# Girjoaba/simplex_method_gpu

Hardware: AMD Instinct MI355X
Metric: simplex iterations/sec on dense m=4096 n=16384 fp64; achieved HBM GB/s (higher is better)
Workload: dtype f64

## Files before the change

include/simplex.h:

```cpp
#ifndef SIMPLEX_MI355X_H
#define SIMPLEX_MI355X_H

#include <stdint.h>

#ifdef __cplusplus
extern "C" {
#endif

#define SPX_ABI_VERSION 8

#define SPX_STATUS_MAX_ITER       0
#define SPX_STATUS_OPTIMUM_FOUND  1
#define SPX_STATUS_UNBOUNDED      2
#define SPX_STATUS_THETA_OVERFLOW 3
#define SPX_STATUS_INFEASIBLE     4

#define SPX_OK             0
#define SPX_ERR_ARG       -1
#define SPX_ERR_HIP       -2
#define SPX_ERR_OOM       -3
#define SPX_ERR_RCCL      -4
#define SPX_ERR_STATE     -5
#define SPX_ERR_NO_DEVICE -6
#define SPX_ERR_SINGULAR  -7
// ... 181 lines not shown

#define SPX_LOOP_FIELDS 7
int spx_loop_times(spx_ctx* ctx, double out[SPX_LOOP_FIELDS], int64_t* passes);

int spx_info(spx_ctx* ctx, int64_t* m, int64_t* n, int64_t* ld,
             int64_t* local_nonbasic, double* bytes_price, double* bytes_update);

#define SPX_CONFIG_FIELDS 17
int spx_config(spx_ctx* ctx, int32_t out[SPX_CONFIG_FIELDS]);

#define SPX_LOOP_LAYOUT_FIELDS 8
int spx_loop_layout(spx_ctx* ctx, int32_t out[SPX_LOOP_LAYOUT_FIELDS]);

int spx_ftran_cols(spx_ctx* ctx, int32_t* cols);

#define SPX_DISPATCH_FIELDS 10
int spx_dispatch_stats(spx_ctx* ctx, int64_t out[SPX_DISPATCH_FIELDS]);

int spx_prepare(spx_ctx* ctx);

int spx_shard_range(int64_t m, int64_t n, int32_t rank, int32_t nranks, int64_t out[4]);
int spx_minloc_merge(const double* vals, const int64_t* idx, int32_t count,
                     double* best_val, int64_t* best_idx);

const char* spx_last_error(void);
const char* spx_status_string(int32_t status);
int spx_abi_version(void);

#ifdef __cplusplus
}
#endif
// ... 2 lines not shown
```

simplex_method_gpu_amd/__init__.py:

```python
from __future__ import annotations

import ctypes
from dataclasses import dataclass
from enum import IntEnum
from typing import NamedTuple

import numpy as np

from ._lib import SimplexError, SpxOpts, check, load

__all__ = ["SolveStatus", "SolveResult", "Context", "solve", "read_lp", "comm_unique_id",
           "shard_range", "minloc_merge", "group_iterate", "group_sync", "check_ranks",
           "SimplexError", "FLAG_TIMING", "RATIO_REFERENCE", "RATIO_GUARDED", "RATIO_HARRIS",
           "PRICING_DANTZIG", "PRICING_DEVEX", "PRICING_STEEPEST", "ALGO_PRIMAL", "ALGO_DUAL",
           "DUAL_PRICING_DANTZIG", "DUAL_PRICING_STEEPEST", "FLAG_DUAL_STEEPEST",
           "DUAL_RATIO_TEXTBOOK", "DUAL_RATIO_LONG_STEP", "FLAG_DUAL_LONG_STEP", "ALGO_PRIMAL_BOX",
           "FLAG_PRIMAL_PHASE1", "PRIMAL_PRICING_DANTZIG", "PRIMAL_PRICING_STEEPEST", "FLAG_PRIMAL_STEEPEST",
           "PRIMAL_WEIGHTS_REFERENCE", "PRIMAL_WEIGHTS_EXACT", "FLAG_PRIMAL_EXACT_WEIGHTS",
           "CostRanging", "RhsRanging"]

FLAG_TIMING = 1
FLAG_STAMPS = 2
FLAG_GLOBAL_Y = 4
FLAG_ROW_SHARD = 8
# ... 496 lines not shown
    def info(self):
        m, n, ld, nb = ctypes.c_int64(), ctypes.c_int64(), ctypes.c_int64(), ctypes.c_int64()
        bp, bu = ctypes.c_double(), ctypes.c_double()
        check(self._L.spx_info(self._h, ctypes.byref(m), ctypes.byref(n), ctypes.byref(ld), ctypes.byref(nb),
                               ctypes.byref(bp), ctypes.byref(bu)))
        return {"m": m.value, "n": n.value, "ld": ld.value, "local_nonbasic": nb.value,
                "bytes_price": bp.value, "bytes_update": bu.value}


    def ftran_cols(self) -> int:
        v = ctypes.c_int32()
        check(self._L.spx_ftran_cols(self._h, ctypes.byref(v)))
        return v.value

    def dispatch_stats(self):
        out = (ctypes.c_int64 * 10)()
        check(self._L.spx_dispatch_stats(self._h, out))
        keys = ("eager_passes", "graph_launches", "graph_passes", "persistent_launches", "persistent_passes",
                "folds", "window_pos", "window", "persist_fallbacks", "graph_builds")
        return dict(zip(keys, list(out)))

    def config(self):
        out = (ctypes.c_int32 * 17)()
        check(self._L.spx_config(self._h, out))
        keys = ("window", "price_block", "price_grid", "price_lds", "update_block", "update_rows", "update_grid",
                "graph_batch", "persistent", "loop_block", "tableau", "loop_grid", "defer_tail", "compact_fold",
                "ftran_rows_per_wave", "mbox_fused", "compact_price")
        cfg = dict(zip(keys, list(out)))
        cfg["dual_pricing"] = self._dual_pricing
        cfg["primal_pricing"] = self._primal_pricing
        cfg["dual_ratio"] = self._dual_ratio
        cfg["primal_weights"] = self._primal_weights
        return cfg

    def loop_layout(self):
        out = (ctypes.c_int32 * 8)()
        check(self._L.spx_loop_layout(self._h, out))
        keys = ("dual_price_lds", "dual_update_lds", "dual_se_update_lds", "dual_se_rho_lds", "pbox_price_lds",
                "pbox_update_lds", "pbox_se_lds_vecs", "slack_unit")
        return dict(zip(keys, list(out)))


def solve(A_cols, b, c, max_iter: int = (1 << 62), eps: float = 1e-7, device: int = -1,
# ... 4 lines not shown
```

simplex_method_gpu_amd/csrc/spx_api.cpp:

```cpp
#include <algorithm>
#include <cmath>
#include <cstdarg>
#include <cstdio>
#include <cstdlib>
#include <cstring>
#include <string>
#include <vector>

#include "spx_ctx.h"
#include "spx_tableau.h"

using namespace spx;
using namespace spx_host;

namespace {

thread_local std::string g_err;

}

int spx_host::fail(int code, const char* fmt, ...) {
    char buf[512];
    va_list ap;
    va_start(ap, fmt);
// ... 403 lines not shown
    HIP_TRY(launch_reset(x->P, x->stream));
    SPX_TRY(box_sync(x));
    HIP_TRY(launch_se_init(x->P, x->stream));
    if (x->P.bc) {
        HIP_TRY(hipMemsetAsync(x->P.rleft, 0, (size_t)x->L * sizeof(int32_t), x->stream));
        HIP_TRY(hipMemsetAsync(x->P.rmap, 0xFF, (size_t)x->L * sizeof(int32_t), x->stream));
        HIP_TRY(hipMemsetAsync(x->P.bc_n, 0, BC_N_WORDS * sizeof(int32_t), x->stream));
        if (x->P.as_off) HIP_TRY(hipMemsetAsync(x->P.as_off, 0, 65 * sizeof(int32_t), x->stream));
    }
    SPX_TRY(tab_rebuild(x, true));
    HIP_TRY(hipStreamSynchronize(x->stream));
    x->pivots = 0;
    x->status = SPX_STATUS_MAX_ITER;
    x->stepped_price = false;
    x->nw = 0;
    x->dw_ok = false;
    x->s_list = 0;
    x->cp_now = x->cp_ok;
    return SPX_OK;
}

bool fold_due(const spx_ctx* x) { return x->P.win && x->nw >= x->P.win; }
void advance_window(spx_ctx* x, bool folded) {
    if (x->P.win) x->nw = (folded ? 1 : x->nw) + 1;
}

int fold_events(spx_ctx* x, hipEvent_t* f0, hipEvent_t* f1) {
    if (x->ev_fold.size() < 2 * (x->n_fold + 1)) {
        for (int i = 0; i < 2; ++i) {
            hipEvent_t e;
            HIP_TRY(hipEventCreate(&e));
// ... 8 lines not shown

int enqueue_pass(spx_ctx* x, bool timed) {
    hipEvent_t p0 = nullptr, p1 = nullptr, u0 = nullptr, u1 = nullptr;
    if (timed) SPX_TRY(pass_events(x, &p0, &p1, &u0, &u1));
    const bool fold = fold_due(x);
    if (x->capturing) x->graph_folds += fold ? 1 : 0;
    else {
        ++x->n_eager;
        x->n_folds += fold ? 1 : 0;
    }
    if (fold) {
        hipEvent_t f0 = nullptr, f1 = nullptr;
        if (timed) SPX_TRY(fold_events(x, &f0, &f1));
        if (x->defer_tail) HIP_TRY(launch_apply_tail(x->P, x->stream));
        if (f0) HIP_TRY(hipEventRecord(f0, x->stream));
        HIP_TRY(launch_fold(x->P, x->P.win, x->cus, x->stream));
        if (f1) HIP_TRY(hipEventRecord(f1, x->stream));
        x->dw_ok = false;
    }
    const bool cp_open = x->cp_now && !x->dw_ok && (fold || x->nw <= 1);
    const bool cp_pass = x->cp_now && x->dw_ok;
    advance_window(x, fold);
    HIP_TRY(launch_se_prep(x->P, x->stream, (x->se_fuse && x->se_chain && !fold) ? x->ucfg.grid : 0));
    Params Pp = x->P;
    Pp.se_fused = x->se_fuse ? 1 : 0;
    Pp.defer_price = x->defer_ok ? 1 : 0;
    Pp.defer_tail = x->defer_tail ? 1 : 0;
    Pp.mbox_fused = (x->mbox_ready && x->mbox_fused) ? 1 : 0;
    if (cp_pass) Pp.price_grid = x->ccfg.grid;
    HIP_TRY(launch_price(Pp, cp_pass ? x->ccfg : (cp_open ? x->dcfg : x->pcfg), x->stream, p0, p1));
    if (cp_open) {
        HIP_TRY(launch_dw_basic(Pp, x->stream));
        x->dw_ok = true;
    }
    if (x->use_comm) {
        if (x->mbox_ready) {
            if (!Pp.mbox_fused) HIP_TRY(launch_exchange(x->P, x->stream));
        } else {
            if (!x->comm_ready) return fail(SPX_ERR_STATE, "nranks > 1 but neither spx_attach_comm nor spx_mbox_attach was called");
            NCCL_TRY(ncclAllGather(x->send, x->recv, sizeof(ArgMinEntry) * x->P.pr_stride, ncclUint8, x->comm,
                                   x->stream));
        }
    }
    if (timed) HIP_TRY(hipEventRecord(x->ev_xend[x->n_price - 1], x->stream));
    HIP_TRY(launch_update(Pp, x->ucfg, x->stream, u0, u1));
    x->se_chain = x->se_fuse;
    if (x->P.split_tail) HIP_TRY(launch_tail(x->P, x->ucfg.grid, x->stream));
    if (x->P.row_shard) {
        if (!x->comm_ready) return fail(SPX_ERR_STATE, "row-sharded B^-1 needs spx_attach_comm");
        NCCL_TRY(ncclAllGather(x->P.rs_send, x->rs_recv, (size_t)x->P.rs_stride, ncclUint8, x->comm, x->stream));
        HIP_TRY(launch_finalize_rs(x->P, x->stream));
    }
    return SPX_OK;
}

int build_graph(spx_ctx* x) {
    hipGraphExec_t& gexec = x->cp_now ? x->graph_exec_c : x->graph_exec;
    hipGraph_t& gkeep = x->cp_now ? x->graph_c : x->graph;
    if (gexec || x->batch <= 0) return SPX_OK;
    if (x->use_comm && !x->comm_ready && !x->mbox_ready)
        return fail(SPX_ERR_STATE, "nranks > 1 but neither spx_attach_comm nor spx_mbox_attach was called");
    HIP_TRY(hipStreamBeginCapture(x->stream, hipStreamCaptureModeThreadLocal));
    int rc = SPX_OK;
    const int nw_keep = x->nw;
    const bool dw_keep = x->dw_ok;
    if (x->P.win) x->nw = x->P.win;
    x->capturing = true;
    x->graph_folds = 0;
    for (int i = 0; i < x->batch && rc == SPX_OK; ++i) rc = enqueue_pass(x, false);
    x->capturing = false;
    x->se_chain = false;
    x->nw = nw_keep;
    x->dw_ok = dw_keep;
    hipGraph_t g = nullptr;
    hipError_t e = hipStreamEndCapture(x->stream, &g);
    hipError_t ei = hipSuccess;
    if (rc == SPX_OK && e == hipSuccess) ei = hipGraphInstantiate(&gexec, g, nullptr, nullptr, 0);
    if (x->use_comm && (rc != SPX_OK || e != hipSuccess || ei != hipSuccess)) {
        if (g) (void)hipGraphDestroy(g);
        gexec = nullptr;
        x->batch = 0;
        x->graph_fallback = true;
        (void)hipGetLastError();
        return SPX_OK;
    }
    if (rc != SPX_OK) return rc;
    if (e != hipSuccess) return fail(SPX_ERR_HIP, "hipStreamEndCapture: %s", hipGetErrorString(e));
    gkeep = g;
    if (ei != hipSuccess) return fail(SPX_ERR_HIP, "hipGraphInstantiate: %s", hipGetErrorString(ei));
    ++x->n_graph_builds;
    HIP_TRY(hipGraphUpload(gexec, x->stream));
    HIP_TRY(hipStreamSynchronize(x->stream));
    return SPX_OK;
}

int build_graphs(spx_ctx* x) {
    if (!x->cp_ok) return build_graph(x);
    const bool keep = x->cp_now;
    const int64_t built = x->n_graph_builds;
    int rc = SPX_OK;
    for (int mode = 1; mode >= 0 && rc == SPX_OK; --mode) {
        x->cp_now = mode != 0;
        rc = build_graph(x);
    }
    x->cp_now = keep;
    if (x->n_graph_builds > built) x->n_graph_builds = built + 1;
    return rc;
}

int check_tickets(spx_ctx* x) {
    bool bad = x->st_host->uncovered != 0;
    if (!bad && x->P.price_dyn && (x->pcfg.wm == 2 || x->pcfg.tk)) {
        uint32_t t[TICKET_WORDS];
        HIP_TRY(hipMemcpy(t, x->P.tickets, sizeof(t), hipMemcpyDeviceToHost));
        for (int k = 0; k < 2 * x->P.tk_shards; ++k) bad = bad || t[32 * k + 1] > t[32 * k];
    }
    if (bad) {
        return fail(SPX_ERR_STATE, "pricing: ticketed list slots were left unpriced (tk_shards %d, grid %d): the "
// ... 119 lines not shown
    if (x->algo == SPX_ALGO_DUAL) return iterate_dual(x, k);
    if (x->algo == SPX_ALGO_PRIMAL_BOX) return iterate_pbox(x, k);
    if (x->persist && !x->stepped_price) {
        SPX_TRY(set_limit(x, x->pivots + k));
        return iterate_persist(x, k);
    }
    if (x->stepped_price) return fail(SPX_ERR_STATE, "spx_price was called without spx_pivot");
    if (!x->cp_ok) return iterate_passes(x, k);
    int64_t left = k;
    while (left > 0 && x->status == SPX_STATUS_MAX_ITER) {
        const int64_t room = (int64_t)x->P.as_cap - x->s_list - x->nw;
        const bool cp = room >= 16;
        const int64_t chunk = cp ? std::min(left, room) : left;
        if (cp != x->cp_now) {
            x->cp_now = cp;
            x->dw_ok = false;
        }
        const int64_t before = x->pivots;
        SPX_TRY(iterate_passes(x, chunk));
        left -= chunk;
        if (x->pivots == before) break;
    }
    return SPX_OK;
}

int iterate_passes(spx_ctx* x, int64_t k) {
    SPX_TRY(set_limit(x, x->pivots + k));
    x->se_chain = false;
    int64_t left = k;
    if (x->batch > 0) {
        const int64_t lead = x->P.win ? std::max(0, x->P.win - x->nw) : 0;
        if (left >= lead + x->batch) {
            for (int64_t i = 0; i < lead; ++i) SPX_TRY(enqueue_pass(x, x->timing));
            left -= lead;
            SPX_TRY(build_graph(x));
            hipGraphExec_t gexec = x->cp_now ? x->graph_exec_c : x->graph_exec;
            const int64_t reps = left / x->batch;
            for (int64_t i = 0; i < reps; ++i) HIP_TRY(hipGraphLaunch(gexec, x->stream));
            if (reps > 0 && x->cp_now) x->dw_ok = true;
            x->se_chain = false;
            x->n_graph_launch += reps;
            x->n_graph_pass += reps * x->batch;
            x->n_folds += reps * x->graph_folds;
            left -= reps * x->batch;
        }
    }
    for (int64_t i = 0; i < left; ++i) SPX_TRY(enqueue_pass(x, x->timing));
    if (x->defer_tail) HIP_TRY(launch_apply_tail(x->P, x->stream));
    x->se_chain = false;
    return read_state(x);
}

int rv_prepare(spx_ctx* x) {
    if (x->rv.X) return SPX_OK;
    RvParams& R = x->rv;
    const int64_t m = x->m, L = x->L;
    R.A = x->A;
    R.m = m;
// ... 64 lines not shown
        return fail(SPX_ERR_SINGULAR, "singular basis: no pivot above tolerance for column %lld (basis position %lld)",
                    (long long)basis[rs.bad_pos], (long long)rs.bad_pos);
    HIP_TRY(rv_launch_finish(x->P, R, x->rv_Ypart, x->stream));
    if (x->P.bc) {
        std::vector<int32_t> left((size_t)x->L, 0);
        for (int64_t k = 0; k < m; ++k) left[(size_t)k] = basis[k] != ns + k ? 1 : 0;
        HIP_TRY(hipMemcpyAsync(x->P.rleft, left.data(), (size_t)x->L * sizeof(int32_t), hipMemcpyHostToDevice,
                               x->stream));
        HIP_TRY(hipMemsetAsync(x->P.rmap, 0xFF, (size_t)x->L * sizeof(int32_t), x->stream));
        HIP_TRY(hipMemsetAsync(x->P.bc_n, 0, BC_N_WORDS * sizeof(int32_t), x->stream));
        HIP_TRY(launch_compact(x->P, x->stream));
        HIP_TRY(hipStreamSynchronize(x->stream));
    }
    SPX_TRY(tab_rebuild(x, false));
    x->nw = 0;
    x->dw_ok = false;
    dual_on_reinvert(x);
    SPX_TRY(pbox_on_reinvert(x));
    return read_state(x);
}

int check_basis(const spx_ctx* x, const int64_t* basis) {
    if (!basis) return fail(SPX_ERR_ARG, "basis is NULL");
    std::vector<char> seen((size_t)x->n, 0);
    for (int64_t k = 0; k < x->m; ++k) {
        const int64_t j = basis[k];
        if (j < 0 || j >= x->n) return fail(SPX_ERR_ARG, "basis[%lld] = %lld out of range", (long long)k, (long long)j);
        if (seen[(size_t)j]) return fail(SPX_ERR_ARG, "column %lld repeated in the basis", (long long)j);
        seen[(size_t)j] = 1;
    }
    return SPX_OK;
// ... 96 lines not shown
    cc.tk = false;
    cc.lds_bytes = (size_t)(cc.block / 64) * sizeof(PricePartial) + 16 + (size_t)round_up(cap, 2) * 16;
    x->dcfg = x->pcfg;
    x->dcfg.dw = true;
    int per_cu = 0, per_cu_d = 0;
    HIP_TRY(price_prepare(cc, &per_cu));
    HIP_TRY(price_prepare(x->dcfg, &per_cu_d));
    const int waves = cc.block / 64;
    cc.grid = (int)std::max<int64_t>(1, std::min<int64_t>({(x->max_local_cols + waves - 1) / waves,
                                                           (int64_t)x->cus * std::max(per_cu, 1), P.price_cap}));
    if (x->opts.price_grid > 0) cc.grid = (int)std::min<int64_t>(x->opts.price_grid, P.price_cap);
    P.as_ld = cap;
    P.as_cap = (int32_t)cap;
    P.AS = static_cast<double*>(d);
    x->cp_ok = x->cp_now = true;
    return SPX_OK;
}

int create_tail(spx_ctx* x) {
    SPX_TRY(do_reset(x));
    if (x->algo == SPX_ALGO_DUAL) return dual_setup(x);
    if (x->algo == SPX_ALGO_PRIMAL_BOX) return pbox_setup(x);
    if (!x->use_comm && !x->persist) SPX_TRY(build_graphs(x));
    return SPX_OK;
}

}

namespace spx_host {

// ... 50 lines not shown
    if (x->status == ST_HANDOFF_TIMEOUT) return fail(SPX_ERR_STATE, "internal error: ratio-test hand-off timed out");
    if (x->status == ST_CPRICE_STATE)
        return fail(SPX_ERR_STATE, "internal error: compact pricing without its rows of A or a valid dw (list %d, rows %d)",
                    x->s_list, x->P.as_cap);
    SPX_TRY(check_tickets(x));
    return SPX_OK;
}

int flush(spx_ctx* x) {
    if (x->stepped_price) return fail(SPX_ERR_STATE, "state readback between spx_price and spx_pivot");
    SPX_TRY(pbox_fresh_y(x));
    if (x->P.win) {
        HIP_TRY(launch_fold(x->P, 2, x->cus, x->stream));
        HIP_TRY(launch_tab_binv(x->P, x->stream));
        x->nw = std::min(x->nw, 1);
        x->dw_ok = false;
    }
    HIP_TRY(launch_flush(x->P, x->stream));
    return SPX_OK;
}

int set_limit(spx_ctx* x, int64_t limit) {
    *x->limit_host = limit;
    HIP_TRY(hipMemcpyAsync(&x->P.st->limit, x->limit_host, sizeof(int64_t), hipMemcpyHostToDevice, x->stream));
    return SPX_OK;
}

int set_running(spx_ctx* x) {
    SPX_TRY(read_state(x));
    const int32_t run = ST_RUNNING;
    HIP_TRY(hipMemcpy(&x->P.st->status, &run, sizeof(run), hipMemcpyHostToDevice));
// ... 57 lines not shown
        spx_destroy(x);
        g_err = keep;
        return rc;
    }
    *out = x;
    return SPX_OK;
}

void spx_destroy(spx_ctx* x) {
    if (!x) return;
    if (x->stream) (void)hipStreamSynchronize(x->stream);
    if (x->graph_exec) (void)hipGraphExecDestroy(x->graph_exec);
    if (x->graph) (void)hipGraphDestroy(x->graph);
    if (x->graph_exec_c) (void)hipGraphExecDestroy(x->graph_exec_c);
    if (x->graph_c) (void)hipGraphDestroy(x->graph_c);
    for (hipEvent_t e : {x->ev_sent, x->ev_recv, x->ev_sent2, x->ev_recv2})
        if (e) (void)hipEventDestroy(e);
    for (hipEvent_t e : x->ev_price) (void)hipEventDestroy(e);
    for (hipEvent_t e : x->ev_update) (void)hipEventDestroy(e);
    for (hipEvent_t e : x->ev_xend) (void)hipEventDestroy(e);
    for (hipEvent_t e : x->ev_loop) (void)hipEventDestroy(e);
    for (hipEvent_t e : x->ev_fold) (void)hipEventDestroy(e);
    for (hipEvent_t e : x->pbox.ev_vtb) (void)hipEventDestroy(e);
    for (hipEvent_t e : x->pbox.ev_wx) (void)hipEventDestroy(e);
    for (const std::vector<hipEvent_t>& v : x->rng.ev)
        for (hipEvent_t e : v) (void)hipEventDestroy(e);
    if (x->comm) (void)ncclCommDestroy(x->comm);
    for (void* p : x->mbox_opened) (void)hipIpcCloseMemHandle(p);
    for (void* p : x->allocs) (void)hipFree(p);
    if (x->st_host) (void)hipHostFree(x->st_host);
// ... 237 lines not shown
        }
    }
    if (cs[0]->status == SPX_STATUS_MAX_ITER && k > 0) {
        for (int g = 0; g < G; ++g) {
            HIP_TRY(hipSetDevice(cs[g]->device));
            SPX_TRY(set_limit(cs[g], cs[g]->pivots + k));
            cs[g]->se_chain = false;
        }
        for (int64_t it = 0; it < k; ++it) {
            for (int g = 0; g < G; ++g) {
                spx_ctx* x = cs[g];
                HIP_TRY(hipSetDevice(x->device));
                const bool fold = fold_due(x);
                if (fold && x->defer_tail) HIP_TRY(launch_apply_tail(x->P, x->stream));
                if (fold) HIP_TRY(launch_fold(x->P, x->P.win, x->cus, x->stream));
                advance_window(x, fold);
                HIP_TRY(launch_se_prep(x->P, x->stream, (x->se_fuse && x->se_chain && !fold) ? x->ucfg.grid : 0));
                ++x->n_eager;
                x->n_folds += fold ? 1 : 0;
                Params Pp = x->P;
                Pp.defer_tail = x->defer_tail ? 1 : 0;
                HIP_TRY(launch_price(Pp, x->pcfg, x->stream, nullptr, nullptr));
                HIP_TRY(hipEventRecord(x->ev_sent, x->stream));
            }
            for (int h = 0; h < G; ++h) {
                spx_ctx* x = cs[h];
                HIP_TRY(hipSetDevice(x->device));
                const int ps = x->P.pr_stride;
                for (int g = 0; g < G; ++g) {
                    HIP_TRY(hipStreamWaitEvent(x->stream, cs[g]->ev_sent, 0));
// ... 204 lines not shown
    if (z) SPX_TRY(spx_objective(x, z));
    SPX_TRY(spx_get_state(x, x_b, b_ixs, nullptr, nullptr, nullptr, status, pivots));
    return SPX_OK;
}

int spx_price(spx_ctx* x, int64_t* p, double* min_e, int32_t* optimal) {
    if (!x) return fail(SPX_ERR_ARG, "ctx is NULL");
    if (x->algo == SPX_ALGO_DUAL)
        return fail(SPX_ERR_STATE, "spx_price / spx_pivot step the primal loop only (the context runs SPX_ALGO_DUAL)");
    if (x->algo == SPX_ALGO_PRIMAL_BOX)
        return fail(SPX_ERR_STATE, "spx_price / spx_pivot step the primal loop only (the context runs SPX_ALGO_PRIMAL_BOX)");
    if (x->status != SPX_STATUS_MAX_ITER) return fail(SPX_ERR_STATE, "solve already terminated");
    SPX_TRY(set_limit(x, x->pivots + 1));
    const bool fold = fold_due(x);
    if (fold) HIP_TRY(launch_fold(x->P, x->P.win, x->cus, x->stream));
    if (fold) x->dw_ok = false;
    ++x->n_eager;
    x->n_folds += fold ? 1 : 0;
    HIP_TRY(launch_se_prep(x->P, x->stream));
    SPX_TRY(clear_tickets(x));
    HIP_TRY(launch_price(x->P, x->pcfg, x->stream, nullptr, nullptr));
    const int ps = x->P.pr_stride;
    if (x->use_comm) {
        if (x->mbox_ready) {
            HIP_TRY(launch_exchange(x->P, x->stream));
        } else {
            if (!x->comm_ready) return fail(SPX_ERR_STATE, "nranks > 1 but neither spx_attach_comm nor spx_mbox_attach was called");
            NCCL_TRY(ncclAllGather(x->send, x->recv, sizeof(ArgMinEntry) * ps, ncclUint8, x->comm, x->stream));
        }
    }
    std::vector<ArgMinEntry> cand((size_t)x->opts.nranks * ps);
// ... 36 lines not shown
    return SPX_OK;
}

int spx_dispatch_stats(spx_ctx* x, int64_t out[SPX_DISPATCH_FIELDS]) {
    if (!x || !out) return fail(SPX_ERR_ARG, "NULL argument");
    out[0] = x->n_eager;
    out[1] = x->n_graph_launch;
    out[2] = x->n_graph_pass;
    out[3] = x->n_persist_launch;
    out[4] = x->n_persist_pass;
    out[5] = x->n_folds;
    out[6] = x->P.win ? x->nw : 0;
    out[7] = x->P.win;
    out[8] = x->n_persist_fallback;
    out[9] = x->n_graph_builds;
    return SPX_OK;
}

int spx_prepare(spx_ctx* x) {
    if (!x) return fail(SPX_ERR_ARG, "ctx is NULL");
    if (x->persist) return SPX_OK;
    if (x->algo != SPX_ALGO_PRIMAL) return SPX_OK;
    return build_graphs(x);
}

int spx_pass_times(spx_ctx* x, double out[3], int64_t* passes) {
    if (!x || !out) return fail(SPX_ERR_ARG, "NULL argument");
    HIP_TRY(hipStreamSynchronize(x->stream));
    double tp = 0.0, tx = 0.0, tu = 0.0;
    for (size_t i = 0; i < x->n_price; ++i) {
// ... 97 lines not shown
    if (ld) *ld = x->L;
    if (local_nb) *local_nb = x->st_host->nb_count;
    int64_t streamed = x->st_host->nb_count;
    if (x->P.slack_unit) {
        std::vector<int64_t> bix((size_t)x->m);
        HIP_TRY(hipMemcpy(bix.data(), x->P.b_ixs, (size_t)x->m * sizeof(int64_t), hipMemcpyDeviceToHost));
        int64_t basic_slacks = 0;
        for (int64_t j : bix) basic_slacks += (j >= x->P.k_lo && j < x->P.k_hi) ? 1 : 0;
        streamed -= (x->P.k_hi - x->P.k_lo) - basic_slacks;
    }
    if (bp) *bp = 8.0 * (double)(x->m + 1) * (double)streamed;
    if (bp && x->cp_ok && x->cp_now && x->P.win > 2) {
        const double kw = (double)x->P.win;
        const double per_col = 8.0 * ((double)x->s_list + 2.0 + 0.5 * (kw - 1.0) + 1.0);
        const double compact = per_col * (double)x->st_host->nb_count;
        *bp = ((kw - 2.0) * compact + *bp) / (kw - 1.0);
    }
    int32_t cols = 0;
    SPX_TRY(spx_ftran_cols(x, &cols));
    const double md = (double)x->m;
    const double fold = (x->P.bc && x->P.cfold) ? 8.0 * md * (3.0 * cols + x->P.win) : 16.0 * md * md;
    if (bu) *bu = x->P.win ? 8.0 * md * (double)cols + fold / (x->P.win - 1) : 16.0 * md * md;
    return SPX_OK;
}

int spx_ftran_cols(spx_ctx* x, int32_t* cols) {
    if (!x || !cols) return fail(SPX_ERR_ARG, "NULL argument");
    *cols = (int32_t)x->m;
    if (x->P.win && x->P.bc) {
        HIP_TRY(hipStreamSynchronize(x->stream));
        HIP_TRY(hipMemcpy(cols, x->P.bc_n, sizeof(int32_t), hipMemcpyDeviceToHost));
    }
    return SPX_OK;
}

int spx_config(spx_ctx* x, int32_t out[SPX_CONFIG_FIELDS]) {
// ... 40 lines not shown
```

simplex_method_gpu_amd/csrc/spx_ctx.h:

```cpp
#pragma once
#include <hip/hip_runtime.h>
#include <rccl/rccl.h>

#include <algorithm>
#include <cstdint>
#include <vector>

#include "../../include/simplex.h"
#include "spx_device.h"
#include "spx_dual.h"
#include "spx_kernels.h"
#include "spx_loop.h"
#include "spx_pbox.h"
#include "spx_ranging.h"
#include "spx_reinv.h"

namespace spx_host {

int fail(int code, const char* fmt, ...);

}

#define HIP_TRY(expr)                                                                          \
    do {                                                                                       \
        hipError_t e_ = (expr);                                                                \
// ... 94 lines not shown
    bool graph_fallback = false;
    uint64_t* mbox = nullptr;
    uint32_t* mbox_seq = nullptr;
    uint64_t** mbox_peer = nullptr;
    std::vector<void*> mbox_opened;
    bool mbox_ready = false;
    bool mbox_fused = false;
    bool bc_want = false;
    bool slack_ident = false;
    bool defer_ok = false;
    bool defer_tail = false;
    bool se_fuse = false;
    bool se_chain = false;
    int64_t se_rows = 0;

    bool cp_ok = false, cp_now = false, dw_ok = false;
    spx::PriceCfg ccfg{}, dcfg{};
    int32_t s_list = 0;
    int32_t* bcn_host = nullptr;

    hipGraphExec_t graph_exec = nullptr;
    hipGraph_t graph = nullptr;
    hipGraphExec_t graph_exec_c = nullptr;
    hipGraph_t graph_c = nullptr;
    int batch = 0;

    hipEvent_t ev_sent = nullptr, ev_recv = nullptr, ev_sent2 = nullptr, ev_recv2 = nullptr;
    int64_t mb = 0;
    unsigned char* rs_recv = nullptr;

    bool timing = false;
    std::vector<hipEvent_t> ev_price, ev_update;
    std::vector<hipEvent_t> ev_xend;
    size_t n_price = 0, n_update = 0;

    int64_t pivots = 0;
    int32_t status = SPX_STATUS_MAX_ITER;
    bool stepped_price = false;
    int nw = 0;
// ... 88 lines not shown
```

simplex_method_gpu_amd/csrc/spx_foldk.hip:

```cpp
#include <hip/hip_runtime.h>
#include <math.h>

#include "spx_device.h"
#include "spx_common.h"
#include "spx_fold.h"
#include "spx_kernels.h"
#include "spx_tableau.h"

namespace spx {

template <int KW>
__global__ __launch_bounds__(FOLD_THREADS) void k_fold(Params P, int min_nw) {
    DevState* st = P.st;
    const int nw = st->nw;
    if (nw < min_nw || nw < 2) return;
    const int nf = nw - 1;
    __shared__ double Rl[KW][FOLD_RP];
    __shared__ double NT[KW][FOLD_NP<KW>];
    __shared__ int s_last;
    const int tid = threadIdx.x, lane = tid & 63;
    const int wave = __builtin_amdgcn_readfirstlane(tid >> 6);
    const int64_t L = P.L;
    const int64_t c0 = (int64_t)blockIdx.x * 64;
    int64_t i0, i1;
// ... 29 lines not shown
            P.xw[i] += d;
        }
    }
    __syncthreads();
    if (tid == 0) {
        s_last = arrive_last(arrive_group(P.arrive, ARR_FOLD), gridDim.x * gridDim.y,
                             blockIdx.y * gridDim.x + blockIdx.x);
    }
    __syncthreads();
    if (s_last && tid == 0) {
        P.SY[0] = P.SY[nf];
        st->nw = 1;
    }
}

__global__ __launch_bounds__(1024) void k_bc_list(Params P, int min_nw) {
    __shared__ int s_w[16];
    __shared__ int s_base;
    const int tid = threadIdx.x, lane = tid & 63, wave = tid >> 6;
    if (min_nw > 0) {
        const int nw = P.st->nw;
        if (nw < min_nw || nw < 2) return;
    }
    if (tid == 0) {
        s_base = P.bc_n[0];
        P.bc_n[3] = P.bc_n[0];
        P.bc_n[4] = P.bc_n[1];
        P.bc_n[5] = 0;
    }
    __syncthreads();
    for (int64_t k0 = 0; k0 < P.m; k0 += 1024) {
        const int64_t k = k0 + tid;
        const bool nu = k < P.m && P.rleft[k] != 0 && P.rmap[k] < 0;
        const uint64_t bal = __ballot(nu);
        const int pre = __popcll(bal & ((1ull << lane) - 1ull));
        if (lane == 0) s_w[wave] = __popcll(bal);
        __syncthreads();
        int off = s_base, tot = 0;
        for (int w = 0; w < 16; ++w) {
            if (w < wave) off += s_w[w];
            tot += s_w[w];
        }
        if (nu) {
            P.rmap[k] = off + pre;
            P.rlist[off + pre] = (int32_t)k;
        }
        __syncthreads();
        if (tid == 0) s_base += tot;
        __syncthreads();
    }
    if (tid == 0) {
        P.bc_n[0] = s_base;
        P.bc_n[1] = s_base > 0 ? ((s_base + 63) / 64) * 64 : 64;
    }
}
__global__ __launch_bounds__(256) void k_as_rows(Params P, int min_nw) {
    if (min_nw > 0) {
        const int nw = P.st->nw;
        if (nw < min_nw || nw < 2) return;
    }
    const int S0 = P.bc_n[3];
    const int S = P.bc_n[0] < P.as_cap ? P.bc_n[0] : P.as_cap;
    const int64_t j = (int64_t)blockIdx.x * 4 + (threadIdx.x >> 6);
    if (j >= P.n) return;
    for (int c = S0 + (int)(threadIdx.x & 63); c < S; c += 64)
        P.AS[j * P.as_ld + c] = P.A[j * P.L + P.rlist[c]];
}
__global__ __launch_bounds__(1024) void k_as_order(Params P, int min_nw) {
    __shared__ int s_row[4096];
    if (min_nw > 0) {
        const int nw = P.st->nw;
        if (nw < min_nw || nw < 2) return;
    }
    const int S = P.bc_n[0] < P.as_cap ? P.bc_n[0] : P.as_cap;
    const int tid = threadIdx.x;
    for (int c = tid; c < S; c += 1024) s_row[c] = P.rlist[c];
    __syncthreads();
    auto key = [](int r) { return (int64_t)((r >> 1) & 63) << 32 | (int64_t)r; };
    for (int c = tid; c < S; c += 1024) {
        const int64_t kc = key(s_row[c]);
        int rank = 0;
        for (int d = 0; d < S; ++d) rank += key(s_row[d]) < kc ? 1 : 0;
        P.as_ord[rank] = c;
    }
    if (tid < 65) {
        int off = 0;
        for (int d = 0; d < S; ++d) off += ((s_row[d] >> 1) & 63) < tid ? 1 : 0;
        P.as_off[tid] = off;
    }
}
static void launch_as_rows(const Params& P, int min_nw, hipStream_t s) {
    if (!P.AS) return;
    hipLaunchKernelGGL(k_as_rows, dim3((unsigned)((P.n + 3) / 4)), dim3(256), 0, s, P, min_nw);
    hipLaunchKernelGGL(k_as_order, dim3(1), dim3(1024), 0, s, P, min_nw);
}

constexpr int BC_ROWS = 4;
__global__ __launch_bounds__(256) void k_bc_gather(Params P) {
    const int S = P.bc_n[0];
    const int64_t L = P.L, ldc = P.bc_n[1];
    double* const bc = bc_buf(P, P.bc_n[2]);
    for (int r = 0; r < BC_ROWS; ++r) {
        const int64_t i = (int64_t)blockIdx.x * BC_ROWS + r;
        if (i >= P.m) break;
        for (int c = threadIdx.x; c < S; c += 256) bc[i * ldc + c] = P.B0[i * L + P.rlist[c]];
    }
}
hipError_t launch_compact(const Params& P, hipStream_t s) {
    if (!P.bc) return hipSuccess;
    hipLaunchKernelGGL(k_bc_list, dim3(1), dim3(1024), 0, s, P, 0);
    launch_as_rows(P, 0, s);
    hipLaunchKernelGGL(k_bc_gather, dim3((unsigned)((P.m + BC_ROWS - 1) / BC_ROWS)), dim3(256), 0, s, P);
    return hipGetLastError();
}

template <int KW>
__device__ __forceinline__ void cfold_tile_issue(const double* Bo, int64_t ldo, int S0, const double* U, int64_t c0,
                                                 int64_t r0, int64_t i1, FoldTilePre<KW>& t) {
    const int lane = threadIdx.x & 63;
    const int kr = lane >> 4, cl = lane & 15;
    const int64_t ilast = i1 > 0 ? i1 - 1 : 0;
#pragma unroll
    for (int r = 0; r < 4; ++r) {
        const int64_t i0r = r0 + kr + 4 * r;
        const int64_t i = i0r < ilast ? i0r : ilast;
#pragma unroll
// ... 208 lines not shown
        }
        if (fsx) fsx[6] = rtime();
    }
    __syncthreads();
    if (fst) fst[4] = rtime();
    if (tid == 0) s_last = arrive_last(arrive_group(P.arrive, ARR_FOLD), gridDim.x, blockIdx.x);
    __syncthreads();
    if (fst) fst[5] = rtime();
    if (s_last && tid == 0) {
        P.SY[0] = P.SY[nf];
        P.bc_n[2] = sel ^ 1;
        st->nw = 1;
    }
}

hipError_t launch_cfold(const Params& P, int min_nw, int cus, hipStream_t s) {
    hipLaunchKernelGGL(k_bc_list, dim3(1), dim3(1024), 0, s, P, min_nw);
    launch_as_rows(P, min_nw, s);
    const int64_t ngmax = P.L / 64;
    const int64_t nc = cus > 0 ? cus : 256;
    const dim3 grid((unsigned)(nc > ngmax ? nc : ngmax));
    switch (P.win) {
        case 8: hipLaunchKernelGGL(k_cfold<8>, grid, dim3(FOLD_THREADS), 0, s, P, min_nw); break;
        case 16: hipLaunchKernelGGL(k_cfold<16>, grid, dim3(FOLD_THREADS), 0, s, P, min_nw); break;
        case 32: hipLaunchKernelGGL(k_cfold<32>, grid, dim3(FOLD_THREADS), 0, s, P, min_nw); break;
        case 64: hipLaunchKernelGGL(k_cfold<64>, grid, dim3(FOLD_THREADS), 0, s, P, min_nw); break;
        default: return hipErrorInvalidValue;
    }
    return hipGetLastError();
}

hipError_t launch_fold(const Params& P, int min_nw, int cus, hipStream_t s) {
    if (P.bc && P.cfold) return launch_cfold(P, min_nw, cus, s);
    if (P.tab) {
        const hipError_t e = launch_tab_fold(P, min_nw, cus, s);
        if (e != hipSuccess) return e;
        if (P.tab_slack) return hipSuccess;
    }
    const int nx = (int)(P.L / 64);
    const dim3 grid((unsigned)nx, (unsigned)fold_grid_y(P.m, nx, cus));
    switch (P.win) {
        case 8: hipLaunchKernelGGL(k_fold<8>, grid, dim3(FOLD_THREADS), 0, s, P, min_nw); break;
        case 16: hipLaunchKernelGGL(k_fold<16>, grid, dim3(FOLD_THREADS), 0, s, P, min_nw); break;
        case 32: hipLaunchKernelGGL(k_fold<32>, grid, dim3(FOLD_THREADS), 0, s, P, min_nw); break;
        case 64: hipLaunchKernelGGL(k_fold<64>, grid, dim3(FOLD_THREADS), 0, s, P, min_nw); break;
        default: return hipErrorInvalidValue;
    }
    const hipError_t e = hipGetLastError();
// ... 6 lines not shown
```

simplex_method_gpu_amd/csrc/spx_kernels.h:

```cpp
#pragma once
#include <hip/hip_runtime.h>

#include "spx_device.h"

namespace spx {

struct PriceCfg {
    int block;
    bool lds_y;
    int wm;
    size_t lds_bytes;
    int grid;
    bool tk = false;
    bool dw = false;
};

struct UpdateCfg {
    int block;
    int rows;
    int grid;
    int bc_entry;
    int mark;
};

// ... 1 lines not shown
hipError_t launch_price(const Params& P, const PriceCfg& c, hipStream_t s, hipEvent_t e0, hipEvent_t e1);
hipError_t launch_dw_basic(const Params& P, hipStream_t s);
hipError_t launch_update(const Params& P, const UpdateCfg& c, hipStream_t s, hipEvent_t e0, hipEvent_t e1);
hipError_t launch_apply_tail(const Params& P, hipStream_t s);
hipError_t launch_generate(double* A, double* b, double* c, int64_t m, int64_t n, int64_t L, uint64_t seed,
                           hipStream_t s);
hipError_t launch_reset(const Params& P, hipStream_t s);
hipError_t launch_flush(const Params& P, hipStream_t s);
hipError_t launch_finalize_rs(const Params& P, hipStream_t s);
hipError_t launch_exchange(const Params& P, hipStream_t s);
hipError_t launch_compact(const Params& P, hipStream_t s);
hipError_t launch_tail(const Params& P, int nparts, hipStream_t s);
hipError_t launch_materialize(const Params& P, double* out, hipStream_t s);
hipError_t launch_reduced_costs(const Params& P, double* e, hipStream_t s);
hipError_t launch_objective(const Params& P, hipStream_t s);
hipError_t launch_fold(const Params& P, int min_nw, int cus, hipStream_t s);
hipError_t launch_se_init(const Params& P, hipStream_t s);
hipError_t launch_se_prep(const Params& P, hipStream_t s, int fused_parts = 0);
int se_parts_for(int64_t m);

}
```

Measured before the change: 30420.

## Carry dense-weight vector across folds instead of re-anchoring each window

Adds a DwCarry state machine so the compact-pricing dw vector is updated incrementally during the fold (k_as_rows adds the window contribution) instead of being recomputed by a dense pricing pass after every fold. A full anchor pass now runs only every `period` folds, default 32, settable through the SPX_DW_ANCHOR environment variable. A separate carry graph is captured and chosen at replay time. The aim is to drop the dense A read of the anchor pass, in exchange for extra per-column work in the fold and possible floating-point drift between anchors.

```diff
diff --git a/include/simplex.h b/include/simplex.h
--- a/include/simplex.h
+++ b/include/simplex.h
@@ -219,7 +219,7 @@
 
 int spx_ftran_cols(spx_ctx* ctx, int32_t* cols);
 
-#define SPX_DISPATCH_FIELDS 10
+#define SPX_DISPATCH_FIELDS 12
 int spx_dispatch_stats(spx_ctx* ctx, int64_t out[SPX_DISPATCH_FIELDS]);
 
 int spx_prepare(spx_ctx* ctx);
diff --git a/simplex_method_gpu_amd/__init__.py b/simplex_method_gpu_amd/__init__.py
--- a/simplex_method_gpu_amd/__init__.py
+++ b/simplex_method_gpu_amd/__init__.py
@@ -534,10 +534,10 @@
         return v.value
 
     def dispatch_stats(self):
-        out = (ctypes.c_int64 * 10)()
+        out = (ctypes.c_int64 * 12)()
         check(self._L.spx_dispatch_stats(self._h, out))
         keys = ("eager_passes", "graph_launches", "graph_passes", "persistent_launches", "persistent_passes",
-                "folds", "window_pos", "window", "persist_fallbacks", "graph_builds")
+                "folds", "window_pos", "window", "persist_fallbacks", "graph_builds", "dw_anchors", "dw_carry")
         return dict(zip(keys, list(out)))
 
     def config(self):
@@ -547,6 +547,7 @@
                 "graph_batch", "persistent", "loop_block", "tableau", "loop_grid", "defer_tail", "compact_fold",
                 "ftran_rows_per_wave", "mbox_fused", "compact_price")
         cfg = dict(zip(keys, list(out)))
+        cfg["dw_carry"] = self.dispatch_stats()["dw_carry"]
         cfg["dual_pricing"] = self._dual_pricing
         cfg["primal_pricing"] = self._primal_pricing
         cfg["dual_ratio"] = self._dual_ratio
diff --git a/simplex_method_gpu_amd/csrc/spx_api.cpp b/simplex_method_gpu_amd/csrc/spx_api.cpp
--- a/simplex_method_gpu_amd/csrc/spx_api.cpp
+++ b/simplex_method_gpu_amd/csrc/spx_api.cpp
@@ -441,7 +441,7 @@
     x->status = SPX_STATUS_MAX_ITER;
     x->stepped_price = false;
     x->nw = 0;
-    x->dw_ok = false;
+    x->dwc.invalidate();
     x->s_list = 0;
     x->cp_now = x->cp_ok;
     return SPX_OK;
@@ -480,12 +480,13 @@
         if (timed) SPX_TRY(fold_events(x, &f0, &f1));
         if (x->defer_tail) HIP_TRY(launch_apply_tail(x->P, x->stream));
         if (f0) HIP_TRY(hipEventRecord(f0, x->stream));
-        HIP_TRY(launch_fold(x->P, x->P.win, x->cus, x->stream));
+        const bool carry = x->cp_now && x->P.cfold && x->dwc.fold();
+        if (!carry) x->dwc.invalidate();
+        HIP_TRY(launch_fold(x->P, x->P.win, x->cus, x->stream, carry));
         if (f1) HIP_TRY(hipEventRecord(f1, x->stream));
-        x->dw_ok = false;
-    }
-    const bool cp_open = x->cp_now && !x->dw_ok && (fold || x->nw <= 1);
-    const bool cp_pass = x->cp_now && x->dw_ok;
+    }
+    const bool cp_open = x->cp_now && !x->dwc.ok && (fold || x->nw <= 1);
+    const bool cp_pass = x->cp_now && x->dwc.ok;
     advance_window(x, fold);
     HIP_TRY(launch_se_prep(x->P, x->stream, (x->se_fuse && x->se_chain && !fold) ? x->ucfg.grid : 0));
     Params Pp = x->P;
@@ -497,7 +498,7 @@
     HIP_TRY(launch_price(Pp, cp_pass ? x->ccfg : (cp_open ? x->dcfg : x->pcfg), x->stream, p0, p1));
     if (cp_open) {
         HIP_TRY(launch_dw_basic(Pp, x->stream));
-        x->dw_ok = true;
+        x->dwc.anchor();
     }
     if (x->use_comm) {
         if (x->mbox_ready) {
@@ -520,24 +521,27 @@
     return SPX_OK;
 }
 
-int build_graph(spx_ctx* x) {
-    hipGraphExec_t& gexec = x->cp_now ? x->graph_exec_c : x->graph_exec;
-    hipGraph_t& gkeep = x->cp_now ? x->graph_c : x->graph;
+int build_graph(spx_ctx* x, bool carry_batch = false) {
+    hipGraphExec_t& gexec = !x->cp_now ? x->graph_exec : (carry_batch ? x->graph_exec_k : x->graph_exec_c);
+    hipGraph_t& gkeep = !x->cp_now ? x->graph : (carry_batch ? x->graph_k : x->graph_c);
     if (gexec || x->batch <= 0) return SPX_OK;
     if (x->use_comm && !x->comm_ready && !x->mbox_ready)
         return fail(SPX_ERR_STATE, "nranks > 1 but neither spx_attach_comm nor spx_mbox_attach was called");
     HIP_TRY(hipStreamBeginCapture(x->stream, hipStreamCaptureModeThreadLocal));
     int rc = SPX_OK;
     const int nw_keep = x->nw;
-    const bool dw_keep = x->dw_ok;
+    const spx_host::DwCarry dw_keep = x->dwc;
     if (x->P.win) x->nw = x->P.win;
+    x->dwc.ok = carry_batch;
+    x->dwc.since = 0;
+    if (carry_batch) x->dwc.period = 0;
     x->capturing = true;
     x->graph_folds = 0;
     for (int i = 0; i < x->batch && rc == SPX_OK; ++i) rc = enqueue_pass(x, false);
     x->capturing = false;
     x->se_chain = false;
     x->nw = nw_keep;
-    x->dw_ok = dw_keep;
+    x->dwc = dw_keep;
     hipGraph_t g = nullptr;
     hipError_t e = hipStreamEndCapture(x->stream, &g);
     hipError_t ei = hipSuccess;
@@ -560,6 +564,8 @@
     return SPX_OK;
 }
 
+bool dw_carries(const spx_ctx* x) { return x->cp_ok && x->P.cfold && x->dwc.period != 1; }
+
 int build_graphs(spx_ctx* x) {
     if (!x->cp_ok) return build_graph(x);
     const bool keep = x->cp_now;
@@ -568,6 +574,7 @@
     for (int mode = 1; mode >= 0 && rc == SPX_OK; --mode) {
         x->cp_now = mode != 0;
         rc = build_graph(x);
+        if (rc == SPX_OK && mode != 0 && dw_carries(x)) rc = build_graph(x, true);
     }
     x->cp_now = keep;
     if (x->n_graph_builds > built) x->n_graph_builds = built + 1;
@@ -717,7 +724,7 @@
         const int64_t chunk = cp ? std::min(left, room) : left;
         if (cp != x->cp_now) {
             x->cp_now = cp;
-            x->dw_ok = false;
+            x->dwc.invalidate();
         }
         const int64_t before = x->pivots;
         SPX_TRY(iterate_passes(x, chunk));
@@ -737,14 +744,25 @@
             for (int64_t i = 0; i < lead; ++i) SPX_TRY(enqueue_pass(x, x->timing));
             left -= lead;
             SPX_TRY(build_graph(x));
-            hipGraphExec_t gexec = x->cp_now ? x->graph_exec_c : x->graph_exec;
+            if (x->cp_now && dw_carries(x)) SPX_TRY(build_graph(x, true));
             const int64_t reps = left / x->batch;
-            for (int64_t i = 0; i < reps; ++i) HIP_TRY(hipGraphLaunch(gexec, x->stream));
-            if (reps > 0 && x->cp_now) x->dw_ok = true;
+            for (int64_t i = 0; i < reps; ++i) {
+                hipGraphExec_t gexec = x->graph_exec;
+                if (x->cp_now) {
+                    const bool ca = x->P.cfold && x->graph_exec_k && x->dwc.fits_carry_batch(x->graph_folds);
+                    gexec = ca ? x->graph_exec_k : (x->dwc.fits_anchor_batch() ? x->graph_exec_c : nullptr);
+                }
+                if (!gexec) {
+                    for (int64_t w = 0; w < x->batch; ++w) SPX_TRY(enqueue_pass(x, x->timing));
+                    continue;
+                }
+                HIP_TRY(hipGraphLaunch(gexec, x->stream));
+                if (x->cp_now) x->dwc.replay(x->graph_folds);
+                ++x->n_graph_launch;
+                x->n_graph_pass += x->batch;
+                x->n_folds += x->graph_folds;
+            }
             x->se_chain = false;
-            x->n_graph_launch += reps;
-            x->n_graph_pass += reps * x->batch;
-            x->n_folds += reps * x->graph_folds;
             left -= reps * x->batch;
         }
     }
@@ -839,7 +857,7 @@
     }
     SPX_TRY(tab_rebuild(x, false));
     x->nw = 0;
-    x->dw_ok = false;
+    x->dwc.invalidate();
     dual_on_reinvert(x);
     SPX_TRY(pbox_on_reinvert(x));
     return read_state(x);
@@ -966,6 +984,7 @@
     P.as_cap = (int32_t)cap;
     P.AS = static_cast<double*>(d);
     x->cp_ok = x->cp_now = true;
+    x->dwc.period = P.cfold ? spx_host::dw_period_from(std::getenv("SPX_DW_ANCHOR")) : 1;
     return SPX_OK;
 }
 
@@ -1046,7 +1065,7 @@
         HIP_TRY(launch_fold(x->P, 2, x->cus, x->stream));
         HIP_TRY(launch_tab_binv(x->P, x->stream));
         x->nw = std::min(x->nw, 1);
-        x->dw_ok = false;
+        x->dwc.invalidate();
     }
     HIP_TRY(launch_flush(x->P, x->stream));
     return SPX_OK;
@@ -1134,6 +1153,8 @@
     if (x->graph) (void)hipGraphDestroy(x->graph);
     if (x->graph_exec_c) (void)hipGraphExecDestroy(x->graph_exec_c);
     if (x->graph_c) (void)hipGraphDestroy(x->graph_c);
+    if (x->graph_exec_k) (void)hipGraphExecDestroy(x->graph_exec_k);
+    if (x->graph_k) (void)hipGraphDestroy(x->graph_k);
     for (hipEvent_t e : {x->ev_sent, x->ev_recv, x->ev_sent2, x->ev_recv2})
         if (e) (void)hipEventDestroy(e);
     for (hipEvent_t e : x->ev_price) (void)hipEventDestroy(e);
@@ -1401,6 +1422,7 @@
                 const bool fold = fold_due(x);
                 if (fold && x->defer_tail) HIP_TRY(launch_apply_tail(x->P, x->stream));
                 if (fold) HIP_TRY(launch_fold(x->P, x->P.win, x->cus, x->stream));
+                if (fold) x->dwc.invalidate();
                 advance_window(x, fold);
                 HIP_TRY(launch_se_prep(x->P, x->stream, (x->se_fuse && x->se_chain && !fold) ? x->ucfg.grid : 0));
                 ++x->n_eager;
@@ -1635,7 +1657,7 @@
     SPX_TRY(set_limit(x, x->pivots + 1));
     const bool fold = fold_due(x);
     if (fold) HIP_TRY(launch_fold(x->P, x->P.win, x->cus, x->stream));
-    if (fold) x->dw_ok = false;
+    if (fold) x->dwc.invalidate();
     ++x->n_eager;
     x->n_folds += fold ? 1 : 0;
     HIP_TRY(launch_se_prep(x->P, x->stream));
@@ -1702,6 +1724,8 @@
     out[7] = x->P.win;
     out[8] = x->n_persist_fallback;
     out[9] = x->n_graph_builds;
+    out[10] = x->dwc.anchors;
+    out[11] = (x->cp_ok && x->cp_now && x->dwc.period != 1) ? (x->dwc.period > 0 ? x->dwc.period : -1) : 0;
     return SPX_OK;
 }
 
@@ -1829,12 +1853,14 @@
         const double kw = (double)x->P.win;
         const double per_col = 8.0 * ((double)x->s_list + 2.0 + 0.5 * (kw - 1.0) + 1.0);
         const double compact = per_col * (double)x->st_host->nb_count;
-        *bp = ((kw - 2.0) * compact + *bp) / (kw - 1.0);
+        *bp = spx_host::dw_mean_price_bytes(*bp, compact, x->P.win, x->dwc.period);
     }
     int32_t cols = 0;
     SPX_TRY(spx_ftran_cols(x, &cols));
     const double md = (double)x->m;
-    const double fold = (x->P.bc && x->P.cfold) ? 8.0 * md * (3.0 * cols + x->P.win) : 16.0 * md * md;
+    double fold = (x->P.bc && x->P.cfold) ? 8.0 * md * (3.0 * cols + x->P.win) : 16.0 * md * md;
+    if (x->cp_now && dw_carries(x) && x->P.win > 2)
+        fold += spx_host::dw_carry_bytes(x->n, x->P.win) * (x->dwc.period > 0 ? 1.0 - 1.0 / x->dwc.period : 1.0);
     if (bu) *bu = x->P.win ? 8.0 * md * (double)cols + fold / (x->P.win - 1) : 16.0 * md * md;
     return SPX_OK;
 }
diff --git a/simplex_method_gpu_amd/csrc/spx_ctx.h b/simplex_method_gpu_amd/csrc/spx_ctx.h
--- a/simplex_method_gpu_amd/csrc/spx_ctx.h
+++ b/simplex_method_gpu_amd/csrc/spx_ctx.h
@@ -9,6 +9,7 @@
 #include "../../include/simplex.h"
 #include "spx_device.h"
 #include "spx_dual.h"
+#include "spx_dwcarry.h"
 #include "spx_kernels.h"
 #include "spx_loop.h"
 #include "spx_pbox.h"
@@ -133,7 +134,8 @@
     bool se_chain = false;
     int64_t se_rows = 0;
 
-    bool cp_ok = false, cp_now = false, dw_ok = false;
+    bool cp_ok = false, cp_now = false;
+    spx_host::DwCarry dwc{};
     spx::PriceCfg ccfg{}, dcfg{};
     int32_t s_list = 0;
     int32_t* bcn_host = nullptr;
@@ -142,6 +144,8 @@
     hipGraph_t graph = nullptr;
     hipGraphExec_t graph_exec_c = nullptr;
     hipGraph_t graph_c = nullptr;
+    hipGraphExec_t graph_exec_k = nullptr;
+    hipGraph_t graph_k = nullptr;
     int batch = 0;
 
     hipEvent_t ev_sent = nullptr, ev_recv = nullptr, ev_sent2 = nullptr, ev_recv2 = nullptr;
diff --git a/simplex_method_gpu_amd/csrc/spx_dwcarry.h b/simplex_method_gpu_amd/csrc/spx_dwcarry.h
--- /dev/null
+++ b/simplex_method_gpu_amd/csrc/spx_dwcarry.h
@@ -0,0 +1,51 @@
+#pragma once
+#include <algorithm>
+#include <cstdint>
+#include <cstdlib>
+
+namespace spx_host {
+
+struct DwCarry {
+    int32_t period = 32;
+    int32_t since = 0;
+    bool ok = false;
+    int64_t anchors = 0;
+
+    bool carry_next() const { return ok && (period == 0 || since + 1 < period); }
+    bool fold() {
+        const bool c = carry_next();
+        if (c) ++since;
+        else ok = false;
+        return c;
+    }
+    void anchor() {
+        ok = true;
+        since = 0;
+        ++anchors;
+    }
+    void invalidate() { ok = false; }
+
+    bool fits_anchor_batch() const { return !carry_next(); }
+    bool fits_carry_batch(int nf) const { return ok && (period == 0 || since + nf < period); }
+    void replay(int nf) {
+        for (int i = 0; i < nf; ++i)
+            if (!fold()) anchor();
+    }
+};
+
+inline int32_t dw_period_from(const char* env, int32_t dflt = 32) {
+    if (!env || !*env) return dflt;
+    char* end = nullptr;
+    const long v = std::strtol(env, &end, 10);
+    if (end == env || v < 0) return dflt;
+    return (int32_t)std::min<long>(v, 1 << 30);
+}
+
+inline double dw_mean_price_bytes(double dense, double compact, int win, int32_t period) {
+    const double passes = (double)(win - 1);
+    const double share = period > 0 ? 1.0 / (double)period : 0.0;
+    return ((passes - share) * compact + share * dense) / passes;
+}
+inline double dw_carry_bytes(int64_t n, int win) { return 8.0 * (double)n * (double)(win + 2); }
+
+}
diff --git a/simplex_method_gpu_amd/csrc/spx_foldk.hip b/simplex_method_gpu_amd/csrc/spx_foldk.hip
--- a/simplex_method_gpu_amd/csrc/spx_foldk.hip
+++ b/simplex_method_gpu_amd/csrc/spx_foldk.hip
@@ -67,7 +67,7 @@
     }
 }
 
-__global__ __launch_bounds__(1024) void k_bc_list(Params P, int min_nw) {
+__global__ __launch_bounds__(1024) void k_bc_list(Params P, int min_nw, int carry) {
     __shared__ int s_w[16];
     __shared__ int s_base;
     const int tid = threadIdx.x, lane = tid & 63, wave = tid >> 6;
@@ -79,7 +79,7 @@
         s_base = P.bc_n[0];
         P.bc_n[3] = P.bc_n[0];
         P.bc_n[4] = P.bc_n[1];
-        P.bc_n[5] = 0;
+        P.bc_n[5] = (carry && min_nw > 0 && P.bc_n[5] == 1) ? 2 : 0;
     }
     __syncthreads();
     for (int64_t k0 = 0; k0 < P.m; k0 += 1024) {
@@ -107,19 +107,28 @@
         P.bc_n[1] = s_base > 0 ? ((s_base + 63) / 64) * 64 : 64;
     }
 }
-__global__ __launch_bounds__(256) void k_as_rows(Params P, int min_nw) {
+__global__ __launch_bounds__(256) void k_as_rows(Params P, int min_nw, int carry) {
+    int nw = 0;
     if (min_nw > 0) {
-        const int nw = P.st->nw;
+        nw = P.st->nw;
         if (nw < min_nw || nw < 2) return;
     }
     const int S0 = P.bc_n[3];
     const int S = P.bc_n[0] < P.as_cap ? P.bc_n[0] : P.as_cap;
     const int64_t j = (int64_t)blockIdx.x * 4 + (threadIdx.x >> 6);
     if (j >= P.n) return;
+    if (carry && min_nw > 0 && P.bc_n[5] == 2) {
+        const int lane = (int)(threadIdx.x & 63);
+        const int KW = P.win, nf = nw - 1;
+        double v = 0.0;
+        if (lane < nf && lane < KW) v = mul_nc(P.SY[lane], P.Wt[j * KW + lane]);
+        v = wave_sum(v);
+        if (lane == 0) P.dw[j] += v;
+    }
     for (int c = S0 + (int)(threadIdx.x & 63); c < S; c += 64)
         P.AS[j * P.as_ld + c] = P.A[j * P.L + P.rlist[c]];
 }
-__global__ __launch_bounds__(1024) void k_as_order(Params P, int min_nw) {
+__global__ __launch_bounds__(1024) void k_as_order(Params P, int min_nw, int carry) {
     __shared__ int s_row[4096];
     if (min_nw > 0) {
         const int nw = P.st->nw;
@@ -141,11 +150,12 @@
         for (int d = 0; d < S; ++d) off += ((s_row[d] >> 1) & 63) < tid ? 1 : 0;
         P.as_off[tid] = off;
     }
-}
-static void launch_as_rows(const Params& P, int min_nw, hipStream_t s) {
+    if (carry && min_nw > 0 && tid == 0 && P.bc_n[5] == 2) P.bc_n[5] = 1;
+}
+static void launch_as_rows(const Params& P, int min_nw, int carry, hipStream_t s) {
     if (!P.AS) return;
-    hipLaunchKernelGGL(k_as_rows, dim3((unsigned)((P.n + 3) / 4)), dim3(256), 0, s, P, min_nw);
-    hipLaunchKernelGGL(k_as_order, dim3(1), dim3(1024), 0, s, P, min_nw);
+    hipLaunchKernelGGL(k_as_rows, dim3((unsigned)((P.n + 3) / 4)), dim3(256), 0, s, P, min_nw, carry);
+    hipLaunchKernelGGL(k_as_order, dim3(1), dim3(1024), 0, s, P, min_nw, carry);
 }
 
 constexpr int BC_ROWS = 4;
@@ -161,8 +171,8 @@
 }
 hipError_t launch_compact(const Params& P, hipStream_t s) {
     if (!P.bc) return hipSuccess;
-    hipLaunchKernelGGL(k_bc_list, dim3(1), dim3(1024), 0, s, P, 0);
-    launch_as_rows(P, 0, s);
+    hipLaunchKernelGGL(k_bc_list, dim3(1), dim3(1024), 0, s, P, 0, 0);
+    launch_as_rows(P, 0, 0, s);
     hipLaunchKernelGGL(k_bc_gather, dim3((unsigned)((P.m + BC_ROWS - 1) / BC_ROWS)), dim3(256), 0, s, P);
     return hipGetLastError();
 }
@@ -401,9 +411,10 @@
     }
 }
 
-hipError_t launch_cfold(const Params& P, int min_nw, int cus, hipStream_t s) {
-    hipLaunchKernelGGL(k_bc_list, dim3(1), dim3(1024), 0, s, P, min_nw);
-    launch_as_rows(P, min_nw, s);
+hipError_t launch_cfold(const Params& P, int min_nw, int cus, hipStream_t s, bool carry) {
+    const int cy = (carry && P.AS) ? 1 : 0;
+    hipLaunchKernelGGL(k_bc_list, dim3(1), dim3(1024), 0, s, P, min_nw, cy);
+    launch_as_rows(P, min_nw, cy, s);
     const int64_t ngmax = P.L / 64;
     const int64_t nc = cus > 0 ? cus : 256;
     const dim3 grid((unsigned)(nc > ngmax ? nc : ngmax));
@@ -417,8 +428,8 @@
     return hipGetLastError();
 }
 
-hipError_t launch_fold(const Params& P, int min_nw, int cus, hipStream_t s) {
-    if (P.bc && P.cfold) return launch_cfold(P, min_nw, cus, s);
+hipError_t launch_fold(const Params& P, int min_nw, int cus, hipStream_t s, bool carry) {
+    if (P.bc && P.cfold) return launch_cfold(P, min_nw, cus, s, carry);
     if (P.tab) {
         const hipError_t e = launch_tab_fold(P, min_nw, cus, s);
         if (e != hipSuccess) return e;
diff --git a/simplex_method_gpu_amd/csrc/spx_kernels.h b/simplex_method_gpu_amd/csrc/spx_kernels.h
--- a/simplex_method_gpu_amd/csrc/spx_kernels.h
+++ b/simplex_method_gpu_amd/csrc/spx_kernels.h
@@ -39,7 +39,7 @@
 hipError_t launch_materialize(const Params& P, double* out, hipStream_t s);
 hipError_t launch_reduced_costs(const Params& P, double* e, hipStream_t s);
 hipError_t launch_objective(const Params& P, hipStream_t s);
-hipError_t launch_fold(const Params& P, int min_nw, int cus, hipStream_t s);
+hipError_t launch_fold(const Params& P, int min_nw, int cus, hipStream_t s, bool carry = false);
 hipError_t launch_se_init(const Params& P, hipStream_t s);
 hipError_t launch_se_prep(const Params& P, hipStream_t s, int fused_parts = 0);
 int se_parts_for(int64_t m);
```

New measurement: 31260, median of 6. 1.03x the previous value.
